# JuliaGaussianProcesses/ApproximateGPs.jl

Hardware: NVIDIA B200
Metric: SVGP ELBO+grad points/sec (FP64) (higher is better)
Workload: dtype f64

## Files before the change

approximategps.jl_b200/csrc/agp.cu:

```cuda
#include <dlfcn.h>
#include <nccl.h>
#include <stdarg.h>
#include <stdio.h>
#include <string.h>

#include <algorithm>
#include <string>
#include <vector>

#include "../../include/agp.h"
#include "dense.cuh"
#include "f32sweep.cuh"
#include "gemm.cuh"
#include "kfun.cuh"
#include "laplace.cuh"
#include "sweep.cuh"

using namespace agp;

static thread_local std::string g_err;
static thread_local int32_t g_err_info = 0;
static int32_t fail(int32_t code, const char* fmt, ...) {
  char buf[1024];
  va_list ap;
// ... 419 lines not shown
extern "C" int32_t agp_dataset_upload_f32(agp_dataset* ds, const float* X, int64_t N, int64_t ldx, int32_t layout, const void* y,
                                          int32_t ytype, int32_t location) {
  if (!ds || !X || N < 0 || N > ds->cap) return fail(AGP_ERR_INVALID, "agp_dataset_upload_f32: bad arguments (N=%lld, cap=%lld)", (long long)N, ds ? (long long)ds->cap : -1LL);
  if (layout != AGP_POINT_MAJOR && layout != AGP_FEATURE_MAJOR) return fail(AGP_ERR_INVALID, "unknown layout %d", layout);
  agp_ctx* c = ds->ctx;
  CU(cudaSetDevice(c->device));
  const int D = ds->D;
  if (ldx <= 0) ldx = layout == AGP_POINT_MAJOR ? D : N;
  const int64_t nflt = layout == AGP_POINT_MAJOR ? N * ldx : (int64_t)D * ldx;
  const float* src = X;
  if (location == AGP_HOST && N > 0) {
    OK(ds->stage.ensure((nflt + 1) / 2 + 1));
    CU(cudaMemcpyAsync(ds->stage.p, X, sizeof(float) * nflt, cudaMemcpyHostToDevice, c->stream));
    src = reinterpret_cast<const float*>(ds->stage.p);
  }
  if (N > 0) {
    widen_x_kernel<<<1024, 256, 0, c->stream>>>(src, ldx, layout, ds->X, N, D);
    LAUNCHED(c);
    KCHECK();
  }
  CU(cudaStreamSynchronize(c->stream));
  OK(upload_y(ds, y, N, ytype, location));
  CU(cudaStreamSynchronize(c->stream));
  ds->N = N;
  return AGP_OK;
}

extern "C" int32_t agp_dataset_size(agp_dataset* ds, int64_t* N, int32_t* D) {
  if (!ds) return fail(AGP_ERR_INVALID, "agp_dataset_size: NULL");
  if (N) *N = ds->N;
  if (D) *D = ds->D;
  return AGP_OK;
}
extern "C" int32_t agp_dataset_destroy(agp_dataset* ds) {
  if (!ds) return AGP_OK;
  cudaSetDevice(ds->ctx->device);
  if (ds->X) cudaFree(ds->X);
  if (ds->y) cudaFree(ds->y);
  ds->stage.release();
  delete ds;
  return AGP_OK;
}

template <auto Kernel>
static int32_t ensure_smem(agp_ctx* c, int bytes) {
  static int granted[64] = {0};
  int& g = granted[c->device & 63];
  if (g > bytes) return AGP_OK;
  if (bytes > 0) CU(cudaFuncSetAttribute(Kernel, cudaFuncAttributeMaxDynamicSharedMemorySize, bytes));
  g = bytes + 1;
  return AGP_OK;
}

template <int MODE, int S>
static int32_t launch_trsm_s(agp_ctx* c, const TrsmArgs& a, int tiles_n) {
  using Cfg = StageCfg<A_KM, B_KN>;
  const int Sx = (MODE == TR_KUF_FWD || MODE == TR_KUF_FWD_SCALED) ? kuf_dp(a.kp.D) + 2 : 0;
  const int smem = (S * (Cfg::elems + BK * Sx) + 64 * Sx) * 8 + 16;
  OK((ensure_smem<trsm_kernel<MODE, S>>(c, smem)));
  trsm_kernel<MODE, S><<<tiles_n, NTHREADS, smem, c->stream>>>(a);
  LAUNCHED(c);
  KCHECK();
  return AGP_OK;
}
template <int MODE>
static int32_t launch_trsm(agp_ctx* c, const TrsmArgs& a, int tiles_n);
static bool s1_fused() {
  static const bool fused = getenv("AGP_S1_FUSED") && atoi(getenv("AGP_S1_FUSED")) != 0;
  return fused;
}
static int32_t launch_s1(agp_ctx* c, const TrsmArgs& t1_in, int tiles_n, bool keep = false, bool gen_only = false) {
  if (s1_fused() && !gen_only) return launch_trsm<TR_KUF_FWD>(c, t1_in, tiles_n);
  TrsmArgs t1 = t1_in;
  KufGenArgs g{};
  g.K = keep ? c->Kf.p : t1.X;
  g.DK = (keep && t1.kp.kind != AGP_KERNEL_SE) ? c->DKb.p : nullptr;
  if (keep) t1.RHS = c->Kf.p;
  g.ldx = t1.ldx;
  g.ncols = tiles_n * BN;
  g.pts = t1.pts;
  g.npts = t1.npts;
  g.zsp = t1.zsp;
  g.kp = t1.kp;
  const int D = t1.kp.D;
  const int smem = 0;
  const dim3 grid((g.ncols + KG_COLS - 1) / KG_COLS, t1.nb * BM / KG_ROWS);
#define AGP_KGEN_D(KD)                                                                   \
  {                                                                                      \
    if (D <= 4) kuf_gen_kernel<4, KD><<<grid, KG_COLS, smem, c->stream>>>(g);            \
    else if (D <= 8) kuf_gen_kernel<8, KD><<<grid, KG_COLS, smem, c->stream>>>(g);       \
    else if (D <= 16) kuf_gen_kernel<16, KD><<<grid, KG_COLS, smem, c->stream>>>(g);     \
    else kuf_gen_kernel<32, KD><<<grid, KG_COLS, smem, c->stream>>>(g);                  \
  }
  switch (t1.kp.kind) {
    case AGP_KERNEL_SE: AGP_KGEN_D(AGP_KERNEL_SE) break;
    case AGP_KERNEL_MATERN32: AGP_KGEN_D(AGP_KERNEL_MATERN32) break;
    case AGP_KERNEL_MATERN52: AGP_KGEN_D(AGP_KERNEL_MATERN52) break;
    case AGP_KERNEL_LINEAR: AGP_KGEN_D(AGP_KERNEL_LINEAR) break;
    default: AGP_KGEN_D(AGP_KERNEL_SUM) break;
  }
#undef AGP_KGEN_D
  LAUNCHED(c);
  KCHECK();
  if (gen_only) return AGP_OK;
  return launch_trsm<TR_RHS_FWD_SUMS>(c, t1, tiles_n);
}

template <int MODE>
static int32_t launch_trsm(agp_ctx* c, const TrsmArgs& a, int tiles_n) {
  if ((MODE == TR_KUF_FWD || MODE == TR_KUF_FWD_SCALED) && a.kp.D > 8) return launch_trsm_s<MODE, 3>(c, a, tiles_n);
  return launch_trsm_s<MODE, 4>(c, a, tiles_n);
}

template <int LA, int LB, int S = StageCfg<LA, LB>::stages, class Epi>
static int32_t run_gemm(agp_ctx* c, int tiles_m, int tiles_n, const double* A, int64_t lda, const double* B, int64_t ldb, int K,
                        int kmode, int tmode, const Epi& epi) {
  using Cfg = StageCfg<LA, LB>;
  constexpr int smem_bytes = S * Cfg::bytes;
  GemmArgs g{A, lda, B, ldb, K, kmode, tmode};
  OK((ensure_smem<gemm_kernel<LA, LB, Epi, S>>(c, smem_bytes)));
  dim3 grid(tiles_m, tiles_n);
  if ((kmode == KR_LOWER || kmode == KR_UPPER) && tmode == TS_ALL && tiles_m > 1) {
    static const int env_g = getenv("AGP_SWIZZLE") ? atoi(getenv("AGP_SWIZZLE")) : 0;
    g.swizzle = env_g > 0 ? env_g : std::max(1, c->sms);
    g.tiles_m = tiles_m;
    g.tiles_n = tiles_n;
    grid = dim3(tiles_m * tiles_n, 1);
  }
  gemm_kernel<LA, LB, Epi, S><<<grid, NTHREADS, smem_bytes, c->stream>>>(g, epi);
  LAUNCHED(c);
  KCHECK();
  return AGP_OK;
}

static EpiStore epi_store(double* C, int64_t ldc, bool rowmajor, double alpha = 1.0, double beta = 0.0, int mask = MASK_NONE,
                          double diag_add = 0.0, const double* u = nullptr, const double* v = nullptr, double r1 = 0.0) {
  EpiStore e;
  e.C = C;
  e.ldc = ldc;
  e.rowmajor = rowmajor ? 1 : 0;
  e.alpha = alpha;
  e.beta = beta;
  e.mask = mask;
  e.diag_add = diag_add;
  e.r1u = u;
  e.r1v = v;
  e.r1 = r1;
  return e;
}

static int32_t fill(agp_ctx* c, double* p, int64_t n, double v) {
  if (n <= 0) return AGP_OK;
  if (v == 0.0) {
    CU(cudaMemsetAsync(p, 0, sizeof(double) * n, c->stream));
    return AGP_OK;
  }
  fill_kernel<<<(int)std::min<int64_t>(1024, (n + 255) / 256), 256, 0, c->stream>>>(p, n, v);
  LAUNCHED(c);
  KCHECK();
  return AGP_OK;
}

static int32_t transpose(agp_ctx* c, const double* in, double* out, int n, int64_t ld) {
  dim3 grid(n / 32, n / 32), block(32, 8);
  transpose_kernel<<<grid, block, 0, c->stream>>>(in, out, n, ld);
  LAUNCHED(c);
  KCHECK();
  return AGP_OK;
}

struct StreamSwap {
  agp_ctx* c;
  cudaStream_t saved;
  StreamSwap(agp_ctx* c_, cudaStream_t s) : c(c_), saved(c_->stream) { c->stream = s; }
  ~StreamSwap() { c->stream = saved; }
};
static int32_t blocked_cholesky_v2(agp_ctx* c, double* Kw, double* L, double* Lt, double* Ut, int nb, int64_t ld, int* info, int nvalid);
static int32_t blocked_cholesky(agp_ctx* c, double* Kw, double* L, double* Lt, double* Ut, int nb, int64_t ld, int* info, int nvalid) {
  static const int sched = getenv("AGP_CHOL_SCHED") ? atoi(getenv("AGP_CHOL_SCHED")) : 2;
  if (sched == 2 && nb > 1) return blocked_cholesky_v2(c, Kw, L, Lt, Ut, nb, ld, info, nvalid);
  OK((ensure_smem<potrf_trinv128_kernel>(c, PT_SMEM_BYTES)));
  constexpr int OB = 4;
// ... 916 lines not shown
      i8e::Args g8{Mp, i8e::KM_UPTO_N, 0, 0};
      OK((ensure_smem<i8e::i8emu_gemm_kernel<i8e::EpiE1>>(c, i8e::SMEM_BYTES)));
      i8e::i8emu_gemm_kernel<i8e::EpiE1><<<dim3(Mp / i8e::EN, ncols / i8e::EM, 1), i8e::E_THREADS, i8e::SMEM_BYTES, c->stream>>>(ma, mb, g8, e1);
      LAUNCHED(c);
      KCHECK();
      i8e::colsum_reduce_kernel<<<(ncols + 255) / 256, 256, 0, c->stream>>>(c->sxx_part.p, nparts, ldc, ncols, c->saa.p, c->sam.p);
      LAUNCHED(c);
      KCHECK();
    } else {
      ProfScope ps(c, PC_TRSM_FWD);
      OK(launch_s1(c, t1, tiles_n, grad && kgrad_fast(st)));
    }
    const int64_t plane = (int64_t)Mp * ldc;
    float* fA = reinterpret_cast<float*>(c->fA.p);
    float* fC = reinterpret_cast<float*>(c->fC.p);
    float* fAb = reinterpret_cast<float*>(c->fAb.p);
    float* fAs = reinterpret_cast<float*>(c->fAs.p);
    const int64_t MMf = (int64_t)Mp * Mp;
    const dim3 grid5(ncols / t5::TM, Mp / t5::TN, 1);
    if (st.f32) {
      if (!a_planes_done) {
        ProfScope ps(c, PC_F32_AUX);
        t5::transpose_split_kernel<<<dim3(ncols / 32, Mp / 32), 256, 0, c->stream>>>(c->A.p, ldc, Mp, ncols, fA, fA + plane, Mp);
        LAUNCHED(c);
        KCHECK();
      }
      ProfScope ps(c, PC_GEMM_BTA);
      t5::EpiF2 e2{fC, fC + plane, Mp, c->scc_part.p, ldc};
      t5::Args g{Mp, t5::KM_FROM_N, 0, 0, t5::MnDesc()};
      OK((launch_t5<false, false>(c, grid5, fA, plane, Mp, ncols, reinterpret_cast<float*>(c->fBtc.p), MMf, Mp, Mp, g, e2)));
    } else if (emu_s2 && ncols >= 2048) {
      ProfScope ps(c, PC_GEMM_BTA);
      const int64_t pbytes = (int64_t)Mp * ldc;
      OK(c->q6As.ensure(((int64_t)i8e::S * pbytes + 7) / 8));
      OK(c->sPm.ensure(ldc));
      signed char* qApm = reinterpret_cast<signed char*>(c->q6As.p);
      i8e::transpose_slice_kernel<i8e::S><<<(ncols + 31) / 32, 256, 0, c->stream>>>(c->A.p, ldc, Mp, ncols, qApm, Mp, pbytes, c->sPm.p);
      LAUNCHED(c);
      KCHECK();
      CUtensorMap ma, mb;
      if (!i8e::make_map3(&ma, qApm, Mp, ncols, Mp, pbytes, i8e::EM, i8e::S) ||
          !i8e::make_map3(&mb, reinterpret_cast<signed char*>(c->qBt7.p), Mp, Mp, Mp, MM, i8e::EN, i8e::S))
        return fail(AGP_ERR_CUDA, "cuTensorMapEncodeTiled failed");
      i8e::EpiE2 e2{c->C.p, ldc, c->sPm.p, c->sBt7.p, c->scc_part.p, ldc};
      i8e::Args g8{Mp, i8e::KM_FROM_N, 0, 0};
      OK((ensure_smem<i8e::i8emu_gemm_kernel<i8e::EpiE2>>(c, i8e::SMEM_BYTES)));
      i8e::i8emu_gemm_kernel<i8e::EpiE2><<<dim3(Mp / i8e::EN, ncols / i8e::EM, 1), i8e::E_THREADS, i8e::SMEM_BYTES, c->stream>>>(ma, mb, g8, e2);
      LAUNCHED(c);
      KCHECK();
    } else {
    EpiS2 e2{c->C.p, ldc, c->scc_part.p, ldc};
    {
      ProfScope ps(c, PC_GEMM_BTA);
      OK((run_gemm<A_KM, B_KN>(c, nb, tiles_n, c->Bt_rm.p, Mp, c->A.p, ldc, Mp, KR_UPPER, TS_ALL, e2)));
    }
    }
    PerPointArgs pp{};
    pp.saa = c->saa.p;
    pp.sam = c->sam.p;
    pp.scc_part = c->scc_part.p;
    pp.ldp = ldc;
    pp.nb = st.f32 ? 2 * nb : ((emu_s2 && ncols >= 2048) ? 4 * nb : nb);
    pp.pts = pts;
    pp.y = y ? y + lo : nullptr;
    pp.npts = npts;
    pp.ncols = ncols;
    pp.scale = st.scale;
    pp.mean_const = st.mean_const;
    pp.kp = st.kp;
    pp.lp = st.lp;
    pp.dmu = c->dmu.p;
    pp.dv = c->dv.p;
    pp.mu_out = mu_out ? mu_out + lo : nullptr;
    pp.var_out = var_out ? var_out + lo : nullptr;
    pp.sc_part = c->sc_part.p;
    pp.flag = c->d_flags + 1;
    pp.predict_only = predict ? 1 : 0;
    pp.point0 = c->st.point_base + lo;
    const int pblocks = (ncols + PP_POINTS_PER_BLOCK - 1) / PP_POINTS_PER_BLOCK;
    {
      ProfScope ps(c, PC_PERPOINT);
      perpoint_kernel<<<pblocks, 256, 0, c->stream>>>(pp);
      LAUNCHED(c);
      KCHECK();
      if (predict) continue;
      const int nsc_used = st.kp.kind == AGP_KERNEL_LINEAR ? SC_DS + D : SC_DS;
      scal_reduce_kernel<<<1, 256, 0, c->stream>>>(c->sc_part.p, pblocks, nsc_used, c->red.p + rl.scal);
      LAUNCHED(c);
      KCHECK();
    }
    if (!grad) continue;
    if (st.f32) {
      const bool s5t = st.f32_tc_solve;
      {
        ProfScope ps(c, PC_GEMM_BC);
        t5::Args g{Mp, t5::KM_UPTO_N, 0, 0, t5::MnDesc()};
        if (s5t) {
          t5::EpiF4<true> e4{fA, fA + plane, fAb, fAb + plane, fAs, fAs + plane, Mp, c->dmu.p, c->dv.p, c->mt.p, c->Ab.p, ldc};
          OK((launch_t5<false, false>(c, grid5, fC, plane, Mp, ncols, reinterpret_cast<float*>(c->fBtr.p), MMf, Mp, Mp, g, e4)));
        } else {
          t5::EpiF4<false> e4{fA, fA + plane, fAb, fAb + plane, fAs, fAs + plane, Mp, c->dmu.p, c->dv.p, c->mt.p, c->Ab.p, ldc};
          if (f32_s5_i8()) {
            CU(cudaMemsetAsync(c->sAb.p + ldc, 0, sizeof(double) * ncols, c->stream));
            e4.abmax = c->sAb.p + ldc;
          }
          OK((launch_t5<false, false>(c, grid5, fC, plane, Mp, ncols, reinterpret_cast<float*>(c->fBtr.p), MMf, Mp, Mp, g, e4)));
        }
// ... 1 lines not shown
      if (s5t) {
        ProfScope ps(c, PC_TRSM_BWD);
        t5::EpiF5 e5{c->Ab.p, ldc};
        t5::Args g{Mp, t5::KM_FROM_N, 0, 0, t5::MnDesc()};
        OK((launch_t5<false, false>(c, grid5, fAb, plane, Mp, ncols, reinterpret_cast<float*>(c->fLi.p), MMf, Mp, Mp, g, e5)));
      } else if (f32_s5_i8()) {
        ProfScope ps(c, PC_TRSM_BWD);
        signed char* qAb = reinterpret_cast<signed char*>(c->qAb.p);
        const int64_t pbytes = (int64_t)Mp * ldc;
        i8e::transpose_slice_kernel<i8e::S5_NS><<<(ncols + 31) / 32, 256, 0, c->stream>>>(c->Ab.p, ldc, Mp, ncols, qAb, Mp, pbytes, c->sAb.p, c->sAb.p + ldc);
        LAUNCHED(c);
        KCHECK();
        CUtensorMap ma, mb;
        if (!i8e::make_map3(&ma, qAb, Mp, ncols, Mp, pbytes, i8e::EM, i8e::S5_NS) ||
            !i8e::make_map3(&mb, reinterpret_cast<signed char*>(c->qLi.p), Mp, Mp, Mp, MM, i8e::S5_N, i8e::S5_NS))
          return fail(AGP_ERR_CUDA, "cuTensorMapEncodeTiled failed");
        i8e::EpiE5 e5{c->Ab.p, ldc, c->sAb.p, c->sLi.p};
        i8e::Args g8{Mp, i8e::KM_FROM_N, 0, 0};
        constexpr int sm8 = i8e::Cfg<i8e::S5_NS, i8e::S5_N>::smem_bytes;
        OK((ensure_smem<i8e::i8emu_gemm_kernel<i8e::EpiE5, i8e::S5_NS, i8e::S5_N>>(c, sm8)));
        i8e::i8emu_gemm_kernel<i8e::EpiE5, i8e::S5_NS, i8e::S5_N><<<dim3(Mp / i8e::S5_N, ncols / i8e::EM, 1), i8e::E_THREADS, sm8, c->stream>>>(ma, mb, g8, e5);
        LAUNCHED(c);
        KCHECK();
      } else {
        TrsmArgs t5a{};
        t5a.T = c->Ut.p;
        t5a.ldt = Mp;
        t5a.nb = nb;
        t5a.X = c->Ab.p;
        t5a.ldx = ldc;
        t5a.kp = st.kp;
        ProfScope ps(c, PC_TRSM_BWD);
        OK(launch_trsm<TR_RHS_BWD>(c, t5a, tiles_n));
      }
      {
        ProfScope ps(c, PC_SYRK);
        const int kchunk = (int)round_up((ncols + c->nsplit - 1) / c->nsplit, t5::TM);
        const int nz = (ncols + kchunk - 1) / kchunk;
        t5::EpiF6 e6{c->Gpart.p, Mp};
        t5::Args g{ncols, t5::KM_SPLIT, kchunk, 1, t5::MnDesc()};
        OK((launch_t5<true, true>(c, dim3(Mp / t5::TM, Mp / t5::TN, nz), fAs, plane, Mp, ncols, fA, plane, Mp, ncols, g, e6)));
      }
      {
        ProfScope ps(c, PC_F32_AUX);
        const int slab = 512, nslab = (ncols + slab - 1) / slab;
        t5::gvec_kernel<<<dim3((Mp / 4 + 255) / 256, nslab), 256, 0, c->stream>>>(fA, fA + plane, Mp, Mp, c->dmu.p, ncols, slab, c->gpart.p, Mp);
        LAUNCHED(c);
        KCHECK();
      }
    } else {
    EpiS4 e4{c->A.p, c->Ab.p, c->As.p, ldc, c->dmu.p, c->dv.p, c->mt.p, c->gpart.p, Mp};
    {
      ProfScope ps(c, PC_GEMM_BC);
      OK((run_gemm<A_KM, B_KN>(c, nb, tiles_n, c->Bt_cm.p, Mp, c->C.p, ldc, Mp, KR_LOWER, TS_ALL, e4)));
    }
    TrsmArgs t5a{};
    t5a.T = c->Ut.p;
    t5a.ldt = Mp;
    t5a.nb = nb;
    t5a.X = c->Ab.p;
    t5a.ldx = ldc;
    t5a.kp = st.kp;
    {
      ProfScope ps(c, PC_TRSM_BWD);
      OK(launch_trsm<TR_RHS_BWD>(c, t5a, tiles_n));
    }
    if (st.f64_emu && Mp >= 768 && ncols >= 2048) {
      ProfScope ps(c, PC_SYRK);
      const int64_t ldk = round_up(ncols, 128), pbytes = (int64_t)Mp * ldk;
      OK(c->q6A.ensure(((int64_t)i8e::S * pbytes + 7) / 8));
      OK(c->q6As.ensure(((int64_t)i8e::S * pbytes + 7) / 8));
      OK(c->s6.ensure(4 * (int64_t)Mp));
      double* sA = c->s6.p;
      double* sAs = c->s6.p + Mp;
      unsigned long long* mx = reinterpret_cast<unsigned long long*>(c->s6.p + 2 * Mp);
      CU(cudaMemsetAsync(mx, 0, sizeof(unsigned long long) * 2 * Mp, c->stream));
      const int seg = 8192;
      const dim3 gmx((ncols + seg - 1) / seg, Mp / 8);
      i8e::rowmax_kernel<<<gmx, 256, 0, c->stream>>>(c->A.p, ldc, Mp, ncols, seg, mx);
      i8e::rowmax_kernel<<<gmx, 256, 0, c->stream>>>(c->As.p, ldc, Mp, ncols, seg, mx + Mp);
      signed char* qA = reinterpret_cast<signed char*>(c->q6A.p);
      signed char* qAs = reinterpret_cast<signed char*>(c->q6As.p);
      const dim3 gsl((unsigned)((ldk + 1023) / 1024), Mp);
      i8e::slice_rows2d_kernel<i8e::S><<<gsl, 256, 0, c->stream>>>(c->A.p, ldc, ncols, qA, ldk, pbytes, mx, sA);
      i8e::slice_rows2d_kernel<i8e::S><<<gsl, 256, 0, c->stream>>>(c->As.p, ldc, ncols, qAs, ldk, pbytes, mx + Mp, sAs);
      c->launches += 4;
      KCHECK();
      CUtensorMap ma, mb;
      if (!i8e::make_map3(&ma, qAs, ldk, Mp, ldk, pbytes, i8e::EM, i8e::S) || !i8e::make_map3(&mb, qA, ldk, Mp, ldk, pbytes, i8e::EN, i8e::S))
        return fail(AGP_ERR_CUDA, "cuTensorMapEncodeTiled failed");
      const int kchunk = 16384, nz = (int)((ldk + kchunk - 1) / kchunk);
      if (nz > c->nsplit) return fail(AGP_ERR_ALLOC, "S6 (INT8): %d slabs of G needed, %d allocated", nz, c->nsplit);
      i8e::EpiE6 e6{c->Gpart.p, Mp, sAs, sA};
      i8e::Args g8{(int)ldk, i8e::KM_SPLIT, kchunk, 1};
      OK((ensure_smem<i8e::i8emu_gemm_kernel<i8e::EpiE6>>(c, i8e::SMEM_BYTES)));
      i8e::i8emu_gemm_kernel<i8e::EpiE6><<<dim3(Mp / i8e::EN, Mp / i8e::EM, nz), i8e::E_THREADS, i8e::SMEM_BYTES, c->stream>>>(ma, mb, g8, e6);
      LAUNCHED(c);
      KCHECK();
    } else {
      ProfScope ps(c, PC_SYRK);
      SyrkArgs s{};
      s.As = c->As.p;
      s.A = c->A.p;
      s.ld = ldc;
      s.ncols = ncols;
      s.kchunk = (int)round_up((ncols + c->nsplit - 1) / c->nsplit, BK);
      s.G = c->Gpart.p;
      s.Mp = Mp;
      using Cfg = StageCfg<A_MK, B_NK>;
      OK((ensure_smem<syrk_kernel>(c, Cfg::smem_bytes)));
      dim3 grid(nb * (nb + 1), c->nsplit);
      syrk_kernel<<<grid, NTHREADS, Cfg::smem_bytes, c->stream>>>(s);
      LAUNCHED(c);
      KCHECK();
    }
    }
    {
      ProfScope ps(c, PC_KGRAD);
      if (kgrad_fast(st)) {
        OK(run_kgrad(c, c->Ab.p, ldc, pts, npts, (npts + 2047) / 2048, c->Kf.p, st.kp.kind != AGP_KERNEL_SE ? c->DKb.p : nullptr));
      } else {
        OK(run_kgrad(c, c->Ab.p, ldc, pts, npts, (npts + 2047) / 2048));
      }
    }
  }
  if (predict || !grad) return AGP_OK;
  sum_slices_kernel<<<(Mp + 255) / 256, 256, 0, c->stream>>>(c->gpart.p, (int)(ldc / BN), Mp, Mp, c->red.p + rl.g);
  LAUNCHED(c);
  KCHECK();
  sum_slices_kernel<<<1024, 256, 0, c->stream>>>(c->Gpart.p, c->nsplit, MM, MM, c->red.p + rl.G);
  LAUNCHED(c);
  KCHECK();
  OK(finish_kgrad(c, c->nslab, 1.0, c->red.p + rl.dZ, c->red.p + rl.theta));
  return AGP_OK;
}

static int32_t check_dataset(agp_ctx* c, agp_dataset* ds, int64_t offset, int64_t count, int D) {
  if (!c || !ds) return fail(AGP_ERR_INVALID, "NULL context or dataset");
  if (ds->ctx != c) return fail(AGP_ERR_INVALID, "dataset belongs to another context");
  if (ds->D != D) return fail(AGP_ERR_INVALID, "dataset dimension %d != params.D %d", ds->D, D);
  const int64_t min_count = (c->comm && c->nranks > 1) ? 0 : 1;
  if (offset < 0 || count < min_count || offset + count > ds->N)
    return fail(AGP_ERR_INVALID, "points [%lld, %lld) outside the dataset (N=%lld)", (long long)offset, (long long)(offset + count), (long long)ds->N);
  return AGP_OK;
}

extern "C" int32_t agp_svgp_sweep(agp_ctx* c, agp_dataset* ds, int64_t offset, int64_t count, const agp_svgp_params* p,
                                  double num_data, int64_t global_batch, int32_t want_grad) {
  if (!c || !p) return fail(AGP_ERR_INVALID, "agp_svgp_sweep: NULL argument");
  if (c->comm && c->nranks > 1 && global_batch <= 0)
    return fail(AGP_ERR_INVALID, "with a communicator attached global_batch (the batch size summed over all ranks) is required: "
                                 "num_data / count of one shard would scale the ELBO by the number of ranks");
  OK(check_dataset(c, ds, offset, count, p->D));
  {
    ProfScope ps(c, PC_PREPARE);
    OK(prepare_step(c, p));
  }
  SvgpState& st = c->st;
  const int64_t gb = global_batch > 0 ? global_batch : count;
  st.scale = (num_data > 0 ? num_data : (double)gb) / (double)gb;
  st.want_grad = want_grad;
  st.point_base = offset + ((long long)c->rank << 40);
  OK(sweep_points(c, ds->X + offset * ds->D, ds->y + offset, count, want_grad != 0, false, nullptr, nullptr));
  st.sweep_pending = true;
  return AGP_OK;
// ... 279 lines not shown
    tb.kp = st.kp;
    OK(launch_trsm<TR_RHS_BWD>(c, tb, 1));
    rhs_to_vec_kernel<<<(Mp + 255) / 256, 256, 0, c->stream>>>(c->vec64.p, Mp, c->vec64b.p);
    LAUNCHED(c);
    KCHECK();
    CU(cudaMemcpyAsync(alpha_out, c->vec64b.p, sizeof(double) * M, cudaMemcpyDeviceToHost, c->stream));
  }
  if (Lk_out) CU(cudaMemcpy2DAsync(Lk_out, sizeof(double) * M, c->Lk.p, sizeof(double) * Mp, sizeof(double) * M, M, cudaMemcpyDeviceToHost, c->stream));
  if (B_out) CU(cudaMemcpy2DAsync(B_out, sizeof(double) * M, c->Bt_cm.p, sizeof(double) * Mp, sizeof(double) * M, M, cudaMemcpyDeviceToHost, c->stream));
  return check_step_flags(c, false);
}

extern "C" int32_t agp_svgp_mean_and_var(agp_ctx* c, const agp_svgp_params* p, const double* Xnew, int64_t n, double* mu_out,
                                         double* var_out) {
  if (!c || !p || !Xnew || n < 1) return fail(AGP_ERR_INVALID, "agp_svgp_mean_and_var: bad arguments");
  OK(prepare_step(c, p));
  SvgpState& st = c->st;
  st.scale = 1.0;
  const int D = st.D;
  OK(c->mu_out.ensure(n + BN));
  OK(c->var_out.ensure(n + BN));
  DevBuf xbuf;
  OK(xbuf.ensure((n + BN) * D));
  CU(cudaMemcpyAsync(xbuf.p, Xnew, sizeof(double) * n * D, cudaMemcpyHostToDevice, c->stream));
  int32_t s = sweep_points(c, xbuf.p, nullptr, n, false, true, c->mu_out.p, c->var_out.p);
  if (s == AGP_OK) {
    if (mu_out) cudaMemcpyAsync(mu_out, c->mu_out.p, sizeof(double) * n, cudaMemcpyDeviceToHost, c->stream);
    if (var_out) cudaMemcpyAsync(var_out, c->var_out.p, sizeof(double) * n, cudaMemcpyDeviceToHost, c->stream);
  }
  cudaError_t e = cudaStreamSynchronize(c->stream);
  xbuf.release();
  if (s != AGP_OK) return s;
  if (e != cudaSuccess) return fail(AGP_ERR_CUDA, "mean_and_var: %s", cudaGetErrorString(e));
  return check_step_flags(c, false);
}

static int32_t project_points(agp_ctx* c, const double* X_dev, int n, int ncols, double* Abuf, double* Cbuf, int64_t ldc) {
  SvgpState& st = c->st;
  TrsmArgs t1{};
  t1.T = c->Lt.p;
  t1.ldt = st.Mp;
  t1.nb = st.nb;
  t1.X = Abuf;
  t1.ldx = ldc;
  t1.pts = X_dev;
  t1.npts = n;
  t1.zsp = c->zsp.p;
  t1.mt = c->mt.p;
  t1.saa = c->saa.p;
  t1.sam = c->sam.p;
  t1.kp = st.kp;
  OK(launch_s1(c, t1, ncols / BN));
  EpiS2 e2{Cbuf, ldc, c->scc_part.p, ldc};
  OK((run_gemm<A_KM, B_KN>(c, st.nb, ncols / BN, c->Bt_rm.p, st.Mp, Abuf, ldc, st.Mp, KR_UPPER, TS_ALL, e2)));
  return AGP_OK;
}

constexpr int64_t AGP_MAX_COV_POINTS = 16384;

extern "C" int32_t agp_svgp_mean_and_cov(agp_ctx* c, const agp_svgp_params* p, const double* X1, int64_t n1, const double* X2, int64_t n2,
                                         double* mu1_out, double* cov_out) {
  if (!c || !p || !X1 || n1 < 1 || !cov_out) return fail(AGP_ERR_INVALID, "agp_svgp_mean_and_cov: bad arguments");
  const bool cross = X2 != nullptr;
  if (!cross) n2 = n1;
  if (n2 < 1) return fail(AGP_ERR_INVALID, "agp_svgp_mean_and_cov: bad arguments");
  if (n1 > AGP_MAX_COV_POINTS || n2 > AGP_MAX_COV_POINTS)
    return fail(AGP_ERR_UNSUPPORTED, "full covariances are limited to %lld points per argument (the matrix is dense)", (long long)AGP_MAX_COV_POINTS);
  OK(prepare_step(c, p));
  SvgpState& st = c->st;
  st.scale = 1.0;
  const int D = st.D, Mp = st.Mp;
  const int n1p = (int)round_up(n1, BM), n2p = (int)round_up(n2, BM);
  OK(ensure_sweep_workspace(c, std::max(n1p, n2p), true));
  const int64_t ldc = c->chunk_cols;
  OK(c->px1.ensure((int64_t)n1p * D));
  OK(c->pxs1.ensure((int64_t)n1p * D));
  OK(c->pxn1.ensure(n1p));
  OK(c->pcov.ensure((int64_t)n1p * n2p));
  OK(c->mu_out.ensure(n1p));
  OK(c->var_out.ensure(n1p));
  CU(cudaMemsetAsync(c->px1.p, 0, sizeof(double) * n1p * D, c->stream));
  CU(cudaMemcpyAsync(c->px1.p, X1, sizeof(double) * n1 * D, cudaMemcpyHostToDevice, c->stream));
  KernelParams kx = st.kp;
  kx.M = (int)n1;
  prep_z_kernel<<<(n1p + 127) / 128, 128, 0, c->stream>>>(c->px1.p, c->pxs1.p, c->pxn1.p, nullptr, n1p, kx);
  LAUNCHED(c);
  KCHECK();
  OK(project_points(c, c->px1.p, (int)n1, n1p, c->A.p, c->C.p, ldc));
  if (mu1_out) {
    PerPointArgs pp{};
    pp.saa = c->saa.p;
    pp.sam = c->sam.p;
    pp.scc_part = c->scc_part.p;
    pp.ldp = ldc;
    pp.nb = st.nb;
    pp.pts = c->px1.p;
    pp.npts = (int)n1;
    pp.ncols = n1p;
    pp.scale = 1.0;
    pp.mean_const = st.mean_const;
    pp.kp = st.kp;
    pp.lp = st.lp;
    pp.mu_out = c->mu_out.p;
    pp.var_out = c->var_out.p;
    pp.flag = c->d_flags + 1;
    pp.predict_only = 1;
    perpoint_kernel<<<(n1p + PP_POINTS_PER_BLOCK - 1) / PP_POINTS_PER_BLOCK, 256, 0, c->stream>>>(pp);
// ... 130 lines not shown
```

approximategps.jl_b200/csrc/common.cuh:

```cuda
#pragma once
#include <cuda_runtime.h>
#include <stdint.h>

namespace agp {

constexpr int BM = 128;
constexpr int BN = 64;
constexpr int BK = 16;
constexpr int NTHREADS = 256;
constexpr int PAD = 4;

constexpr int A_KM = 0, A_MK = 1;
constexpr int B_KN = 0, B_NK = 1;

template <int LA>
struct ATile {
  static constexpr int ld = (LA == A_KM) ? (BM + PAD) : (BK + PAD);
  static constexpr int elems = (LA == A_KM) ? BK * (BM + PAD) : BM * (BK + PAD);
};
template <int LB>
struct BTile {
  static constexpr int ld = (LB == B_KN) ? (BN + PAD) : (BK + PAD);
  static constexpr int elems = (LB == B_KN) ? BK * (BN + PAD) : BN * (BK + PAD);
};
// ... 88 lines not shown
template <int LB>
struct BLoad {
  static constexpr int NCH = (BK * BN / 2) / NTHREADS;
  static constexpr int SSTEP = (LB == B_KN) ? (NTHREADS / (BN / 2)) * BTile<LB>::ld : (NTHREADS / (BK / 2)) * BTile<LB>::ld;
  int64_t goff, gstep;
  int soff;
  __device__ __forceinline__ void init(int64_t ldb, int tid) {
    if (LB == B_KN) {
      const int k = tid / (BN / 2), nc = tid % (BN / 2);
      goff = (int64_t)k * ldb + nc * 2;
      gstep = (int64_t)(NTHREADS / (BN / 2)) * ldb;
      soff = k * BTile<LB>::ld + nc * 2;
    } else {
      const int n = tid / (BK / 2), kc = tid % (BK / 2);
      goff = (int64_t)n * ldb + kc * 2;
      gstep = (int64_t)(NTHREADS / (BK / 2)) * ldb;
      soff = n * BTile<LB>::ld + kc * 2;
    }
  }
  __device__ __forceinline__ void load(double* sB, const double* __restrict__ gtile) const {
    const double* g = gtile + goff;
    double* s = sB + soff;
#pragma unroll
    for (int i = 0; i < NCH; i++) cp_async16(s + i * SSTEP, g + i * gstep);
  }
};

struct ThreadMap {
  int warp, lane, g, t, wm, wn;
  __device__ __forceinline__ ThreadMap() {
    int tid = threadIdx.x;
    warp = tid >> 5;
    lane = tid & 31;
    g = lane >> 2;
    t = lane & 3;
    wm = ((warp < 4) ? warp : 3 - (warp & 3)) * 32;
    wn = (warp >> 2) * 32;
  }
  __device__ __forceinline__ bool tri_active_lower(int krel) const { return krel < wm + 32; }
  __device__ __forceinline__ bool tri_active_upper(int krel) const { return krel + BK > wm; }
  __device__ __forceinline__ int row(int mi) const { return wm + mi * 8 + g; }
  __device__ __forceinline__ int col(int ni, int e) const { return wn + ni * 8 + 2 * t + e; }
};

typedef double Acc[4][4][2];

__device__ __forceinline__ void acc_zero(Acc& acc) {
#pragma unroll
  for (int i = 0; i < 4; i++)
#pragma unroll
    for (int j = 0; j < 4; j++) acc[i][j][0] = acc[i][j][1] = 0.0;
}

template <int LA, int LB>
__device__ __forceinline__ void mma_stage(Acc& acc, const double* __restrict__ sA, const double* __restrict__ sB,
                                          const ThreadMap& tm) {
  constexpr int lda = ATile<LA>::ld, ldb = BTile<LB>::ld;
#pragma unroll
  for (int kk = 0; kk < BK; kk += 4) {
    double a[4], b[4];
#pragma unroll
    for (int mi = 0; mi < 4; mi++)
      a[mi] = (LA == A_KM) ? sA[(kk + tm.t) * lda + tm.wm + mi * 8 + tm.g] : sA[(tm.wm + mi * 8 + tm.g) * lda + kk + tm.t];
#pragma unroll
    for (int ni = 0; ni < 4; ni++)
      b[ni] = (LB == B_KN) ? sB[(kk + tm.t) * ldb + tm.wn + ni * 8 + tm.g] : sB[(tm.wn + ni * 8 + tm.g) * ldb + kk + tm.t];
#pragma unroll
    for (int mi = 0; mi < 4; mi++)
#pragma unroll
      for (int ni = 0; ni < 4; ni++) dmma884(acc[mi][ni], a[mi], b[ni]);
  }
}

__device__ __forceinline__ double block_sum(double v, double* sred ) {
#pragma unroll
  for (int o = 16; o > 0; o >>= 1) v += __shfl_xor_sync(0xffffffffu, v, o);
  int warp = threadIdx.x >> 5, lane = threadIdx.x & 31;
  __syncthreads();
  if (lane == 0) sred[warp] = v;
  __syncthreads();
  double r = 0.0;
  if (threadIdx.x == 0) {
    int nw = (blockDim.x + 31) >> 5;
    for (int w = 0; w < nw; w++) r += sred[w];
  }
  return r;
}

}
```

approximategps.jl_b200/csrc/gemm.cuh:

```cuda
#pragma once
#include "common.cuh"

namespace agp {

constexpr int KR_FULL = 0;
constexpr int KR_LOWER = 1;
constexpr int KR_UPPER = 2;
constexpr int KR_DIAG = 3;
constexpr int TS_ALL = 0;
constexpr int TS_NBLK_LT = 1;
constexpr int TS_NBLK_GT = 2;
constexpr int TS_NBLK_LE = 3;
constexpr int TS_NBLK_LE1 = 4;

struct GemmArgs {
  const double* A;
  int64_t lda;
  const double* B;
  int64_t ldb;
  int K;
  int kmode;
  int tmode;
  int swizzle = 0;
  int tiles_m = 0, tiles_n = 0;
};

constexpr int TRI_NONE = 0, TRI_LOWER = 1, TRI_UPPER = 2;

template <int LA, int LB, int S = StageCfg<LA, LB>::stages>
__device__ __forceinline__ void gemm_mainloop(Acc& acc, double* smem, const double* __restrict__ gA, int64_t lda,
                                              const double* __restrict__ gB, int64_t ldb, int nsteps,
                                              const ThreadMap& tm, int tri = TRI_NONE, int diag_step = 0,
                                              bool whole_active = true) {
  using Cfg = StageCfg<LA, LB>;
  const int tid = threadIdx.x;
  const int64_t a_step = (LA == A_KM) ? (int64_t)BK * lda : (int64_t)BK;
  const int64_t b_step = (LB == B_KN) ? (int64_t)BK * ldb : (int64_t)BK;
  ALoad<LA> la;
  BLoad<LB> lb;
  la.init(lda, tid);
  lb.init(ldb, tid);
  const double* pa = gA;
  const double* pb = gB;
#pragma unroll
  for (int s = 0; s < S - 1; s++) {
    if (s < nsteps) {
      double* st = smem + s * Cfg::elems;
      la.load(st, pa);
      lb.load(st + Cfg::a_elems, pb);
      pa += a_step;
      pb += b_step;
    }
    cp_async_commit();
  }
  int slot_issue = S - 1, slot_cons = 0;
  for (int step = 0; step < nsteps; step++) {
    cp_async_wait<S - 2>();
    __syncthreads();
    if (step + S - 1 < nsteps) {
      double* st = smem + slot_issue * Cfg::elems;
      la.load(st, pa);
      lb.load(st + Cfg::a_elems, pb);
      pa += a_step;
      pb += b_step;
    }
    cp_async_commit();
    slot_issue = (slot_issue + 1 == S) ? 0 : slot_issue + 1;
    const double* st = smem + slot_cons * Cfg::elems;
    slot_cons = (slot_cons + 1 == S) ? 0 : slot_cons + 1;
    bool active = whole_active;
    if (tri != TRI_NONE) {
      const int d = step - diag_step;
      if (d >= 0 && d < BM / BK) active = (tri == TRI_LOWER) ? tm.tri_active_lower(d * BK) : tm.tri_active_upper(d * BK);
    }
    if (active) mma_stage<LA, LB>(acc, st, st + Cfg::a_elems, tm);
  }
  cp_async_wait<0>();
  __syncthreads();
}

template <int LA, int LB, class Epi, int S = StageCfg<LA, LB>::stages>
__global__ void __launch_bounds__(NTHREADS, 2) gemm_kernel(GemmArgs g, Epi epi) {
  extern __shared__ __align__(128) double smem[];
  ThreadMap tm;
  int tile_m = blockIdx.x, tile_n = blockIdx.y;
  if (g.swizzle > 0) {
    const int tiles_m = g.tiles_m, tiles_n = g.tiles_n, G = g.swizzle;
    const int id = blockIdx.x;
    const int sg = id / (G * tiles_m);
    const int gw = min(G, tiles_n - sg * G);
    const int r = id - sg * G * tiles_m;
    const int rank = r / gw;
    tile_n = sg * G + r % gw;
    tile_m = (g.kmode == KR_LOWER) ? tiles_m - 1 - rank : rank;
  }
  const int m0 = tile_m * BM, n0 = tile_n * BN;
  const int nblk = n0 / BM;
  if (g.tmode == TS_NBLK_LT && !(nblk < tile_m)) return;
  if (g.tmode == TS_NBLK_GT && !(nblk > tile_m)) return;
  if (g.tmode == TS_NBLK_LE && !(nblk <= tile_m)) return;
  if (g.tmode == TS_NBLK_LE1 && !(nblk <= tile_m + 1)) return;
  int kb = 0, ke = g.K;
  if (g.kmode == KR_LOWER) ke = min(g.K, (tile_m + 1) * BM);
  if (g.kmode == KR_UPPER) kb = tile_m * BM;
  if (g.kmode == KR_DIAG) {
    kb = tile_m * BM;
    ke = kb + BM;
  }
  const double* gA = (LA == A_KM) ? g.A + (int64_t)kb * g.lda + m0 : g.A + (int64_t)m0 * g.lda + kb;
  const double* gB = (LB == B_KN) ? g.B + (int64_t)kb * g.ldb + n0 : g.B + (int64_t)n0 * g.ldb + kb;
  Acc acc;
  acc_zero(acc);
  const int nsteps = (ke - kb) / BK;
  int tri = TRI_NONE, diag_step = 0;
  if (g.kmode == KR_LOWER && ke == (tile_m + 1) * BM) {
    tri = TRI_LOWER;
    diag_step = nsteps - BM / BK;
  } else if (g.kmode == KR_UPPER) {
    tri = TRI_UPPER;
  }
  gemm_mainloop<LA, LB, S>(acc, smem, gA, g.lda, gB, g.ldb, nsteps, tm, tri, diag_step);
  epi(acc, tm, m0, n0, smem);
}

constexpr int MASK_NONE = 0;
constexpr int MASK_LOWER = 1;
constexpr int MASK_PHI = 2;

struct EpiStore {
  double* C;
  int64_t ldc;
  int rowmajor;
  double alpha;
  double beta;
  int mask;
  double diag_add;
  const double* r1u;
  const double* r1v;
  double r1;
  __device__ __forceinline__ void operator()(Acc& acc, const ThreadMap& tm, int m0, int n0, double*) const {
#pragma unroll
    for (int mi = 0; mi < 4; mi++) {
      const int row = m0 + tm.row(mi);
      const double ur = r1u ? r1 * r1u[row] : 0.0;
#pragma unroll
      for (int ni = 0; ni < 4; ni++) {
#pragma unroll
        for (int e = 0; e < 2; e++) {
          const int col = n0 + tm.col(ni, e);
          double* p = rowmajor ? C + (int64_t)row * ldc + col : C + (int64_t)col * ldc + row;
          double v = alpha * acc[mi][ni][e];
          if (beta != 0.0) v += beta * (*p);
          if (r1u) v += ur * r1v[col];
          if (row == col) v += diag_add;
          if (mask != MASK_NONE) {
            if (col > row) v = 0.0;
            if (mask == MASK_PHI && col == row) v *= 0.5;
          }
          *p = v;
        }
      }
    }
  }
};

}
```

approximategps.jl_b200/csrc/sweep.cuh:

```cuda
#pragma once
#include "gemm.cuh"
#include "kfun.cuh"

namespace agp {

constexpr int TR_KUF_FWD = 0, TR_RHS_FWD = 1, TR_RHS_BWD = 2, TR_KUF_FWD_SCALED = 3, TR_RHS_FWD_SUMS = 4;

struct TrsmArgs {
  const double* T;
  int64_t ldt;
  int nb;
  double* X;
  int64_t ldx;
  const double* RHS;
  const double* pts;
  int npts;
  const double* zsp;
  const double* mt;
  double* saa;
  double* sam;
  const double* rowscale;
  const double* dvec;
  double* skd;
  KernelParams kp;
// ... 517 lines not shown
  }
  double v[5] = {E[0] + E[1], dmu[0] + dmu[1], dvar[0] * kf[0] + dvar[1] * kf[1], ds2[0] + ds2[1],
                 linear ? (dvar[0] + dvar[1]) * p.kp.variance : 0.0};
#pragma unroll
  for (int q = 0; q < 5; q++)
#pragma unroll
    for (int o = 16; o > 0; o >>= 1) v[q] += __shfl_xor_sync(0xffffffffu, v[q], o);
  const int warp = threadIdx.x >> 5, lane = threadIdx.x & 31;
  if (lane == 0)
#pragma unroll
    for (int q = 0; q < 5; q++) sred[warp][q] = v[q];
  __syncthreads();
  double* out = p.sc_part + (int64_t)blockIdx.x * NSC;
  if (threadIdx.x < 5) {
    double r = 0.0;
    for (int w = 0; w < 8; w++) r += sred[w][threadIdx.x];
    out[threadIdx.x] = r;
  }
  if (linear) {
    for (int d = 0; d < p.kp.D; d++) {
      double t = 0.0;
#pragma unroll
      for (int h = 0; h < 2; h++)
        if (n0 + h < p.npts) {
          const double x = p.pts[(int64_t)(n0 + h) * p.kp.D + d];
          t += dvar[h] * 2.0 * p.kp.variance * p.kp.s[d] * x * x;
        }
      const double r = block_sum(t, sred1);
      if (threadIdx.x == 0) out[SC_DS + d] = r;
    }
  }
}

__global__ void __launch_bounds__(256) scal_reduce_kernel(const double* part, int nblocks, int nsc_used, double* acc) {
  __shared__ double sred[8];
  for (int j = 0; j < nsc_used; j++) {
    double v = 0.0;
    for (int b = threadIdx.x; b < nblocks; b += blockDim.x) v += part[(int64_t)b * NSC + j];
    const double r = block_sum(v, sred);
    if (threadIdx.x == 0) acc[j] += r;
  }
}

struct SyrkArgs {
  const double* As;
  const double* A;
  int64_t ld;
  int ncols;
  int kchunk;
  double* G;
  int Mp;
};

__global__ void __launch_bounds__(NTHREADS, 2) syrk_kernel(SyrkArgs a) {
  extern __shared__ __align__(128) double smem[];
  ThreadMap tm;
  int t = blockIdx.x, ti = 0;
  while (t >= 2 * ti + 2) {
    t -= 2 * ti + 2;
    ti++;
  }
  const int tj = t;
  const int split = blockIdx.y;
  const int kb = split * a.kchunk;
  const int ke = min(a.ncols, kb + a.kchunk);
  if (kb >= ke) return;
  const int m0 = ti * BM, n0 = tj * BN;
  Acc acc;
  acc_zero(acc);
  const bool needed = m0 + tm.wm + 31 >= n0 + tm.wn;
  gemm_mainloop<A_MK, B_NK>(acc, smem, a.As + (int64_t)m0 * a.ld + kb, a.ld, a.A + (int64_t)n0 * a.ld + kb, a.ld,
                            (ke - kb) / BK, tm, TRI_NONE, 0, needed);
  double* G = a.G + (int64_t)split * a.Mp * a.Mp;
#pragma unroll
  for (int mi = 0; mi < 4; mi++)
#pragma unroll
    for (int ni = 0; ni < 4; ni++)
#pragma unroll
      for (int e = 0; e < 2; e++) G[(int64_t)(n0 + tm.col(ni, e)) * a.Mp + m0 + tm.row(mi)] += acc[mi][ni][e];
}

struct KgradArgs {
  const double* Kb;
  const double* Kf;
  const double* DK;
  int64_t ld;
  const double* pts;
  int npts;
  const double* zs;
  const double* zn;
  int slab;
  double* part;
  int stride;
  int Mp;
  KernelParams kp;
};
__host__ __device__ __forceinline__ int kgrad_stride(int D) { return 2 * D + 3 + 2 * MAXC; }
__host__ __device__ __forceinline__ int theta_size(int D) { return 2 + D + 2 * MAXC; }
constexpr int AGP_KERNEL_COMPOSITE = AGP_KERNEL_SUM;

template <int DMAX, int RW, int KIND>
__global__ void __launch_bounds__(256, (DMAX <= 8 && RW == 1) ? 2 : 1) kgrad_kernel(KgradArgs a) {
  extern __shared__ __align__(16) double kg_smem[];
  const int warp = threadIdx.x >> 5, lane = threadIdx.x & 31;
  const int row0 = (blockIdx.x * 8 + warp) * RW;
  const int slab = blockIdx.y;
  constexpr int kind = KIND;
  const int D = a.kp.D, Dp = (D + 1) & ~1, Sx = Dp + 2;
  const bool direct = D == 1 && kind != AGP_KERNEL_LINEAR;
  const int nb = slab * a.slab, ne = min(a.npts, nb + a.slab);
  double z[RW][DMAX], znr[RW];
  bool rvalid[RW];
#pragma unroll
  for (int r = 0; r < RW; r++) {
    rvalid[r] = row0 + r < a.kp.M;
#pragma unroll
    for (int d = 0; d < DMAX; d++) z[r][d] = (d < D && rvalid[r]) ? a.zs[(int64_t)(row0 + r) * D + d] : 0.0;
    znr[r] = rvalid[r] ? a.zn[row0 + r] : 0.0;
  }
  double rs[RW], dvar[RW], dcc[RW], wx[RW][DMAX], wxx[RW][DMAX];
  constexpr bool composite = KIND == AGP_KERNEL_COMPOSITE;
  double cP[composite ? RW : 1][MAXC], cQ[composite ? RW : 1][MAXC];
#pragma unroll
  for (int c = 0; c < MAXC; c++)
// ... 290 lines not shown
```

Baseline: 5.485 million.

## Add register double-buffered GEMM mainloop and use it for SVGP sweep GEMMs

```diff
diff --git a/approximategps.jl_b200/csrc/agp.cu b/approximategps.jl_b200/csrc/agp.cu
--- a/approximategps.jl_b200/csrc/agp.cu
+++ b/approximategps.jl_b200/csrc/agp.cu
@@ -495,6 +495,11 @@
   return AGP_OK;
 }
 
+static bool mainloop_v1() {
+  const char* e = getenv("AGP_MAINLOOP");
+  return e && strcmp(e, "v1") == 0;
+}
+
 template <int MODE, int S>
 static int32_t launch_trsm_s(agp_ctx* c, const TrsmArgs& a, int tiles_n) {
   using Cfg = StageCfg<A_KM, B_KN>;
@@ -555,13 +560,12 @@
   return launch_trsm_s<MODE, 4>(c, a, tiles_n);
 }
 
-template <int LA, int LB, int S = StageCfg<LA, LB>::stages, class Epi>
+template <int LA, int LB, int S = StageCfg<LA, LB>::stages, int ML = ML_V1, class Epi>
 static int32_t run_gemm(agp_ctx* c, int tiles_m, int tiles_n, const double* A, int64_t lda, const double* B, int64_t ldb, int K,
                         int kmode, int tmode, const Epi& epi) {
   using Cfg = StageCfg<LA, LB>;
   constexpr int smem_bytes = S * Cfg::bytes;
   GemmArgs g{A, lda, B, ldb, K, kmode, tmode};
-  OK((ensure_smem<gemm_kernel<LA, LB, Epi, S>>(c, smem_bytes)));
   dim3 grid(tiles_m, tiles_n);
   if ((kmode == KR_LOWER || kmode == KR_UPPER) && tmode == TS_ALL && tiles_m > 1) {
     static const int env_g = getenv("AGP_SWIZZLE") ? atoi(getenv("AGP_SWIZZLE")) : 0;
@@ -570,7 +574,13 @@
     g.tiles_n = tiles_n;
     grid = dim3(tiles_m * tiles_n, 1);
   }
-  gemm_kernel<LA, LB, Epi, S><<<grid, NTHREADS, smem_bytes, c->stream>>>(g, epi);
+  if (ML == ML_V1 || mainloop_v1()) {
+    OK((ensure_smem<gemm_kernel<LA, LB, Epi, S, ML_V1>>(c, smem_bytes)));
+    gemm_kernel<LA, LB, Epi, S, ML_V1><<<grid, NTHREADS, smem_bytes, c->stream>>>(g, epi);
+  } else {
+    OK((ensure_smem<gemm_kernel<LA, LB, Epi, S, ML>>(c, smem_bytes)));
+    gemm_kernel<LA, LB, Epi, S, ML><<<grid, NTHREADS, smem_bytes, c->stream>>>(g, epi);
+  }
   LAUNCHED(c);
   KCHECK();
   return AGP_OK;
@@ -1593,7 +1603,7 @@
     EpiS2 e2{c->C.p, ldc, c->scc_part.p, ldc};
     {
       ProfScope ps(c, PC_GEMM_BTA);
-      OK((run_gemm<A_KM, B_KN>(c, nb, tiles_n, c->Bt_rm.p, Mp, c->A.p, ldc, Mp, KR_UPPER, TS_ALL, e2)));
+      OK((run_gemm<A_KM, B_KN, StageCfg<A_KM, B_KN>::stages, ML_V2>(c, nb, tiles_n, c->Bt_rm.p, Mp, c->A.p, ldc, Mp, KR_UPPER, TS_ALL, e2)));
     }
     }
     PerPointArgs pp{};
@@ -1701,7 +1711,7 @@
     EpiS4 e4{c->A.p, c->Ab.p, c->As.p, ldc, c->dmu.p, c->dv.p, c->mt.p, c->gpart.p, Mp};
     {
       ProfScope ps(c, PC_GEMM_BC);
-      OK((run_gemm<A_KM, B_KN>(c, nb, tiles_n, c->Bt_cm.p, Mp, c->C.p, ldc, Mp, KR_LOWER, TS_ALL, e4)));
+      OK((run_gemm<A_KM, B_KN, StageCfg<A_KM, B_KN>::stages, ML_V2>(c, nb, tiles_n, c->Bt_cm.p, Mp, c->C.p, ldc, Mp, KR_LOWER, TS_ALL, e4)));
     }
     TrsmArgs t5a{};
     t5a.T = c->Ut.p;
@@ -1757,9 +1767,14 @@
       s.G = c->Gpart.p;
       s.Mp = Mp;
       using Cfg = StageCfg<A_MK, B_NK>;
-      OK((ensure_smem<syrk_kernel>(c, Cfg::smem_bytes)));
       dim3 grid(nb * (nb + 1), c->nsplit);
-      syrk_kernel<<<grid, NTHREADS, Cfg::smem_bytes, c->stream>>>(s);
+      if (mainloop_v1()) {
+        OK((ensure_smem<syrk_kernel<ML_V1>>(c, Cfg::smem_bytes)));
+        syrk_kernel<ML_V1><<<grid, NTHREADS, Cfg::smem_bytes, c->stream>>>(s);
+      } else {
+        OK((ensure_smem<syrk_kernel<ML_V2>>(c, Cfg::smem_bytes)));
+        syrk_kernel<ML_V2><<<grid, NTHREADS, Cfg::smem_bytes, c->stream>>>(s);
+      }
       LAUNCHED(c);
       KCHECK();
     }
@@ -2145,7 +2160,7 @@
   t1.kp = st.kp;
   OK(launch_s1(c, t1, ncols / BN));
   EpiS2 e2{Cbuf, ldc, c->scc_part.p, ldc};
-  OK((run_gemm<A_KM, B_KN>(c, st.nb, ncols / BN, c->Bt_rm.p, st.Mp, Abuf, ldc, st.Mp, KR_UPPER, TS_ALL, e2)));
+  OK((run_gemm<A_KM, B_KN, StageCfg<A_KM, B_KN>::stages, ML_V2>(c, st.nb, ncols / BN, c->Bt_rm.p, st.Mp, Abuf, ldc, st.Mp, KR_UPPER, TS_ALL, e2)));
   return AGP_OK;
 }
 
diff --git a/approximategps.jl_b200/csrc/common.cuh b/approximategps.jl_b200/csrc/common.cuh
--- a/approximategps.jl_b200/csrc/common.cuh
+++ b/approximategps.jl_b200/csrc/common.cuh
@@ -164,24 +164,58 @@
     for (int j = 0; j < 4; j++) acc[i][j][0] = acc[i][j][1] = 0.0;
 }
 
+struct Frag {
+  double a[4], b[4];
+};
+template <int LA, int LB>
+__device__ __forceinline__ void load_frag(Frag& f, const double* __restrict__ sA, const double* __restrict__ sB, int kk,
+                                          const ThreadMap& tm) {
+  constexpr int lda = ATile<LA>::ld, ldb = BTile<LB>::ld;
+#pragma unroll
+  for (int mi = 0; mi < 4; mi++)
+    f.a[mi] = (LA == A_KM) ? sA[(kk + tm.t) * lda + tm.wm + mi * 8 + tm.g] : sA[(tm.wm + mi * 8 + tm.g) * lda + kk + tm.t];
+#pragma unroll
+  for (int ni = 0; ni < 4; ni++)
+    f.b[ni] = (LB == B_KN) ? sB[(kk + tm.t) * ldb + tm.wn + ni * 8 + tm.g] : sB[(tm.wn + ni * 8 + tm.g) * ldb + kk + tm.t];
+}
+__device__ __forceinline__ void mma_frag(Acc& acc, const Frag& f) {
+#pragma unroll
+  for (int mi = 0; mi < 4; mi++)
+#pragma unroll
+    for (int ni = 0; ni < 4; ni++) dmma884(acc[mi][ni], f.a[mi], f.b[ni]);
+}
+
 template <int LA, int LB>
 __device__ __forceinline__ void mma_stage(Acc& acc, const double* __restrict__ sA, const double* __restrict__ sB,
                                           const ThreadMap& tm) {
-  constexpr int lda = ATile<LA>::ld, ldb = BTile<LB>::ld;
 #pragma unroll
   for (int kk = 0; kk < BK; kk += 4) {
-    double a[4], b[4];
-#pragma unroll
-    for (int mi = 0; mi < 4; mi++)
-      a[mi] = (LA == A_KM) ? sA[(kk + tm.t) * lda + tm.wm + mi * 8 + tm.g] : sA[(tm.wm + mi * 8 + tm.g) * lda + kk + tm.t];
-#pragma unroll
-    for (int ni = 0; ni < 4; ni++)
-      b[ni] = (LB == B_KN) ? sB[(kk + tm.t) * ldb + tm.wn + ni * 8 + tm.g] : sB[(tm.wn + ni * 8 + tm.g) * ldb + kk + tm.t];
-#pragma unroll
-    for (int mi = 0; mi < 4; mi++)
-#pragma unroll
-      for (int ni = 0; ni < 4; ni++) dmma884(acc[mi][ni], a[mi], b[ni]);
-  }
+    Frag f;
+    load_frag<LA, LB>(f, sA, sB, kk, tm);
+    mma_frag(acc, f);
+  }
+}
+
+constexpr int ML_V1 = 1, ML_V2 = 2;
+
+template <int LA, int LB>
+__device__ __forceinline__ void v2_substeps(Acc& acc, Frag (&f)[2], const double* __restrict__ sA, const double* __restrict__ sB,
+                                            const ThreadMap& tm, bool active) {
+#pragma unroll
+  for (int j = 0; j < BK / 4 - 1; j++) {
+    load_frag<LA, LB>(f[(j + 1) & 1], sA, sB, 4 * (j + 1), tm);
+    if (active) mma_frag(acc, f[j & 1]);
+  }
+}
+
+template <int LA, int LB, int S, class Refill>
+__device__ __forceinline__ void v2_boundary(Frag& f0, const double* __restrict__ next_sA, const double* __restrict__ next_sB,
+                                            const ThreadMap& tm, Refill&& refill) {
+  cp_async_wait<S - 2>();
+  __syncthreads();
+  refill();
+  cp_async_commit();
+  load_frag<LA, LB>(f0, next_sA, next_sB, 0, tm);
 }
 
 __device__ __forceinline__ double block_sum(double v, double* sred ) {
diff --git a/approximategps.jl_b200/csrc/gemm.cuh b/approximategps.jl_b200/csrc/gemm.cuh
--- a/approximategps.jl_b200/csrc/gemm.cuh
+++ b/approximategps.jl_b200/csrc/gemm.cuh
@@ -27,11 +27,19 @@
 
 constexpr int TRI_NONE = 0, TRI_LOWER = 1, TRI_UPPER = 2;
 
-template <int LA, int LB, int S = StageCfg<LA, LB>::stages>
-__device__ __forceinline__ void gemm_mainloop(Acc& acc, double* smem, const double* __restrict__ gA, int64_t lda,
-                                              const double* __restrict__ gB, int64_t ldb, int nsteps,
-                                              const ThreadMap& tm, int tri = TRI_NONE, int diag_step = 0,
-                                              bool whole_active = true) {
+__device__ __forceinline__ bool stage_active(const ThreadMap& tm, int step, int tri, int diag_step, bool whole_active) {
+  bool active = whole_active;
+  if (tri != TRI_NONE) {
+    const int d = step - diag_step;
+    if (d >= 0 && d < BM / BK) active = (tri == TRI_LOWER) ? tm.tri_active_lower(d * BK) : tm.tri_active_upper(d * BK);
+  }
+  return active;
+}
+
+template <int LA, int LB, int S>
+__device__ __forceinline__ void gemm_mainloop_v2(Acc& acc, double* smem, const double* __restrict__ gA, int64_t lda,
+                                                 const double* __restrict__ gB, int64_t ldb, int nsteps, const ThreadMap& tm,
+                                                 int tri, int diag_step, bool whole_active) {
   using Cfg = StageCfg<LA, LB>;
   const int tid = threadIdx.x;
   const int64_t a_step = (LA == A_KM) ? (int64_t)BK * lda : (int64_t)BK;
@@ -43,6 +51,63 @@
   const double* pa = gA;
   const double* pb = gB;
 #pragma unroll
+  for (int s = 0; s < S; s++) {
+    if (s < nsteps) {
+      double* st = smem + s * Cfg::elems;
+      la.load(st, pa);
+      lb.load(st + Cfg::a_elems, pb);
+      pa += a_step;
+      pb += b_step;
+    }
+    cp_async_commit();
+  }
+  cp_async_wait<S - 1>();
+  __syncthreads();
+  Frag f[2];
+  load_frag<LA, LB>(f[0], smem, smem + Cfg::a_elems, 0, tm);
+  int slot = 0;
+  for (int step = 0; step < nsteps; step++) {
+    const bool active = stage_active(tm, step, tri, diag_step, whole_active);
+    double* st = smem + slot * Cfg::elems;
+    v2_substeps<LA, LB>(acc, f, st, st + Cfg::a_elems, tm, active);
+    if (step + 1 < nsteps) {
+      slot = (slot + 1 == S) ? 0 : slot + 1;
+      const double* nx = smem + slot * Cfg::elems;
+      v2_boundary<LA, LB, S>(f[0], nx, nx + Cfg::a_elems, tm, [&] {
+        if (step + S < nsteps) {
+          la.load(st, pa);
+          lb.load(st + Cfg::a_elems, pb);
+          pa += a_step;
+          pb += b_step;
+        }
+      });
+    }
+    if (active) mma_frag(acc, f[1]);
+  }
+  cp_async_wait<0>();
+  __syncthreads();
+}
+
+template <int LA, int LB, int S = StageCfg<LA, LB>::stages, int ML = ML_V1>
+__device__ __forceinline__ void gemm_mainloop(Acc& acc, double* smem, const double* __restrict__ gA, int64_t lda,
+                                              const double* __restrict__ gB, int64_t ldb, int nsteps,
+                                              const ThreadMap& tm, int tri = TRI_NONE, int diag_step = 0,
+                                              bool whole_active = true) {
+  if constexpr (ML == ML_V2) {
+    gemm_mainloop_v2<LA, LB, S>(acc, smem, gA, lda, gB, ldb, nsteps, tm, tri, diag_step, whole_active);
+    return;
+  }
+  using Cfg = StageCfg<LA, LB>;
+  const int tid = threadIdx.x;
+  const int64_t a_step = (LA == A_KM) ? (int64_t)BK * lda : (int64_t)BK;
+  const int64_t b_step = (LB == B_KN) ? (int64_t)BK * ldb : (int64_t)BK;
+  ALoad<LA> la;
+  BLoad<LB> lb;
+  la.init(lda, tid);
+  lb.init(ldb, tid);
+  const double* pa = gA;
+  const double* pb = gB;
+#pragma unroll
   for (int s = 0; s < S - 1; s++) {
     if (s < nsteps) {
       double* st = smem + s * Cfg::elems;
@@ -68,18 +133,13 @@
     slot_issue = (slot_issue + 1 == S) ? 0 : slot_issue + 1;
     const double* st = smem + slot_cons * Cfg::elems;
     slot_cons = (slot_cons + 1 == S) ? 0 : slot_cons + 1;
-    bool active = whole_active;
-    if (tri != TRI_NONE) {
-      const int d = step - diag_step;
-      if (d >= 0 && d < BM / BK) active = (tri == TRI_LOWER) ? tm.tri_active_lower(d * BK) : tm.tri_active_upper(d * BK);
-    }
-    if (active) mma_stage<LA, LB>(acc, st, st + Cfg::a_elems, tm);
+    if (stage_active(tm, step, tri, diag_step, whole_active)) mma_stage<LA, LB>(acc, st, st + Cfg::a_elems, tm);
   }
   cp_async_wait<0>();
   __syncthreads();
 }
 
-template <int LA, int LB, class Epi, int S = StageCfg<LA, LB>::stages>
+template <int LA, int LB, class Epi, int S = StageCfg<LA, LB>::stages, int ML = ML_V1>
 __global__ void __launch_bounds__(NTHREADS, 2) gemm_kernel(GemmArgs g, Epi epi) {
   extern __shared__ __align__(128) double smem[];
   ThreadMap tm;
@@ -119,7 +179,7 @@
   } else if (g.kmode == KR_UPPER) {
     tri = TRI_UPPER;
   }
-  gemm_mainloop<LA, LB, S>(acc, smem, gA, g.lda, gB, g.ldb, nsteps, tm, tri, diag_step);
+  gemm_mainloop<LA, LB, S, ML>(acc, smem, gA, g.lda, gB, g.ldb, nsteps, tm, tri, diag_step);
   epi(acc, tm, m0, n0, smem);
 }
 
diff --git a/approximategps.jl_b200/csrc/sweep.cuh b/approximategps.jl_b200/csrc/sweep.cuh
--- a/approximategps.jl_b200/csrc/sweep.cuh
+++ b/approximategps.jl_b200/csrc/sweep.cuh
@@ -593,6 +593,7 @@
   int Mp;
 };
 
+template <int ML>
 __global__ void __launch_bounds__(NTHREADS, 2) syrk_kernel(SyrkArgs a) {
   extern __shared__ __align__(128) double smem[];
   ThreadMap tm;
@@ -610,7 +611,7 @@
   Acc acc;
   acc_zero(acc);
   const bool needed = m0 + tm.wm + 31 >= n0 + tm.wn;
-  gemm_mainloop<A_MK, B_NK>(acc, smem, a.As + (int64_t)m0 * a.ld + kb, a.ld, a.A + (int64_t)n0 * a.ld + kb, a.ld,
+  gemm_mainloop<A_MK, B_NK, StageCfg<A_MK, B_NK>::stages, ML>(acc, smem, a.As + (int64_t)m0 * a.ld + kb, a.ld, a.A + (int64_t)n0 * a.ld + kb, a.ld,
                             (ke - kb) / BK, tm, TRI_NONE, 0, needed);
   double* G = a.G + (int64_t)split * a.Mp * a.Mp;
 #pragma unroll
```

Result: no change. 5.539 million, median of 6 (+1.0%).
